# pfnet-research/chainer-differentiable-mpc

Measured on AMD Instinct MI355X. Metric: LQR timestep-solves/sec @ batch=4096 T=50 n_x=8 n_u=2, higher is better.
Workload: dtype f32

## Files before the change

### chainer_differentiable_mpc_amd/csrc/gen_lqr_asm.py

```python
#!/usr/bin/env python
import os

HERE = os.path.dirname(os.path.abspath(__file__))
OUT = os.path.join(HERE, "lqr_asm_gen.hpp")

SHAPES = [(8, 2), (3, 1), (4, 2), (6, 2), (2, 2), (1, 1), (2, 1), (3, 2), (4, 4)]
DB = 3
DF = int(os.environ.get("GEN_FWD_DEPTH", "6"))
KROW = 12
VBASE = 128

X_NO_VMWAIT = os.environ.get("GEN_NO_VMWAIT") == "1"
X_NO_DMA = os.environ.get("GEN_NO_DMA") == "1"
X_NO_LDSREAD = os.environ.get("GEN_NO_LDSREAD") == "1"
X_SKIP_FWD = os.environ.get("GEN_SKIP_FWD") == "1"
X_SKIP_BWD = os.environ.get("GEN_SKIP_BWD") == "1"
X_FWD = set(os.environ.get("GEN_FWD_SKIP", "").split(","))
X_TIMING = os.environ.get("GEN_TIMING") == "1"
X_NEWTON = os.environ.get("GEN_NEWTON") == "1"
X_WARM_STUBS = os.environ.get("GEN_WARM_STUBS") == "1"
X_RET_DIRECT = os.environ.get("GEN_RET_SETPC") != "1"
MFMA_USE = int(os.environ.get("GEN_MFMA_USE", "5"))
MFMA_DEP = int(os.environ.get("GEN_MFMA_DEP", "2"))
X_QP_VALU = os.environ.get("GEN_QP_VALU", "1") == "1"
X_G10_MIX = os.environ.get("GEN_G10_MIX") == "1"
RING_DEPTH = int(os.environ.get("GEN_RING_DEPTH", "3"))
X_NT = set(os.environ.get("GEN_NT", "plain,save,affine,adj").split(","))
USE_MFMA = os.environ.get("GEN_NO_MFMA") != "1"


class Layout:
    def __init__(self, nx, nu, depth=DB, ghbm=False):
        self.nx, self.nu, self.ns = nx, nu, nx + nu
        self.depth = depth
        ns = self.ns
        self.nC, self.nc, self.nF, self.nf = ns * ns, ns, nx * ns, nx
        self.OFF_C = 0
        self.OFF_c = 16 * self.nC
        self.OFF_F = self.OFF_c + 16 * self.nc
        self.OFF_f = self.OFF_F + 16 * self.nF
        self.nchunk_b = self.nC + self.nc + self.nF + self.nf
        self.ndma_b = (self.nchunk_b + 63) // 64
        self.compact = depth > DB
        self.SLOT_B = self.ndma_b * 1024 if not self.compact else (16 * self.nchunk_b + 63) // 64 * 64
        self.last_lanes = (self.SLOT_B - (self.ndma_b - 1) * 1024) // 16
        self.FOFF_f = 16 * self.nF
        self.nG = nu * KROW // 4 * 1 if ghbm else 0
        assert (nu * KROW) % 4 == 0
        self.nG = nu * KROW if ghbm else 0
        self.FOFF_G = 16 * (self.nF + self.nf)
        self.nchunk_f = self.nF + self.nf + self.nG
        self.ndma_f = (self.nchunk_f + 63) // 64
        self.SLOT_F = self.ndma_f * 1024
        deep = RING_DEPTH * ((16 * self.nchunk_b + 63) // 64 * 64) if RING_DEPTH > DB else 0
        self.RING = max(deep, DB * self.ndma_b * 1024, DF * self.SLOT_F)
        assert depth * self.SLOT_B <= self.RING
        assert self.ndma_b * 1024 - 1024 <= 4095 and ns + 1 <= 12 and nu in (1, 2, 3, 4)
        assert (depth - 1) * self.ndma_b <= 63 and (DF - 1) * self.ndma_f <= 63 and 1 <= self.last_lanes <= 64
        self.stash_ok = (64 % nx == 0) and nx <= 8
        self.H = (ns + 1) // 2
        self.stash_pieces = []
        o = 0
        while self.H - o >= 2:
            self.stash_pieces.append((2, o))
            o += 2
        if self.H - o == 1:
            self.stash_pieces.append((1, o))
        self.stash_regs = self.H
        self.NSTASH = min(256 // self.stash_regs - (1 if 256 % self.stash_regs == 0 else 0), 64)
        self.SPD = 64 // nx
        self.NFD = (self.NSTASH + 1 + self.SPD - 1) // self.SPD
        self.FAREA = self.NFD * 1024


# ... 72 lines not shown
                self.trans[w] = 0
            else:
                self.trans.pop(w, None)

    def fmac_dpp(self, acc, a, b, lane):
        self.valu("v_fmac_f32_dpp %s, %s, %s row_newbcast:%d row_mask:0xf bank_mask:0xf" % (acc, a, b, lane),
                  writes=(acc,), reads=(b, acc), dpp=a)

    def mul_dpp(self, dst, a, b, lane):
        self.valu("v_mul_f32_dpp %s, %s, %s row_newbcast:%d row_mask:0xf bank_mask:0xf" % (dst, a, b, lane),
                  writes=(dst,), reads=(b,), dpp=a)

    def mov_dpp(self, dst, a, lane):
        self.valu("v_mov_b32_dpp %s, %s row_newbcast:%d row_mask:0xf bank_mask:0xf" % (dst, a, lane),
                  writes=(dst,), dpp=a)

    def v(self, text, writes=(), reads=(), trans=False):
        self.valu(text, writes=writes, reads=reads, trans=trans)

    def text(self):
        return self.lines


class Regs:
    def __init__(self, base):
        self.next = base

    def take(self, n=1, align=1):
        while self.next % align:
            self.next += 1
        r = list(range(self.next, self.next + n))
        self.next += n
        return ["v%d" % i for i in r]


def vrange(regs):
    a, b = int(regs[0][1:]), int(regs[-1][1:])
    assert b - a + 1 == len(regs)
    return "v[%d:%d]" % (a, b)


def gen_kernel(nx, nu, write_k, stash, masked=False, mpc=False, expand=False, ghbm=False, save=False, affine=False, adj=False):
    D = DB if (masked or mpc) else RING_DEPTH
    kind = "mpc" if mpc else "masked" if masked else "save" if save else "adj" if adj else "affine" if affine else "plain"
    L = Layout(nx, nu, D, ghbm)
    ns, aff = L.ns, L.ns
    assert not stash or L.stash_ok
    assert not ghbm or not (stash or write_k or masked or mpc or save or affine)
    assert not mpc or (masked and write_k and not stash)
    assert not expand or (mpc and 12 * nu + 4 * nx <= 64)
    assert not save or (write_k and not masked and not mpc)
    assert not affine or (stash and not write_k and not masked and not mpc and not save and ns >= 4)
    assert not adj or affine
    P = Prog()
    R = Regs(VBASE)
    ptr = ["%%[ptr%d]" % q for q in range(L.ndma_b)]
    str1 = ["%%[str1_%d]" % q for q in range(L.ndma_b)]
    strd = ["%%[str%d]" % q for q in range(L.ndma_b)]
    aq = ["%%[aq%d]" % i for i in range(ns)]
    af = ["%%[af%d]" % k for k in range(nx)]
    fptr = ["%%[fptr%d]" % q for q in range(2 if adj else L.ndma_f)]
    fstr = ["%%[fstr%d]" % q for q in range(2 if adj else L.ndma_f)]
    fp = ["%%[fp%d]" % q for q in range(L.NFD)]
    pk = ["%%[pk%d]" % m for m in range(nu)]

    mfma = USE_MFMA and ns <= 12 and nx % 4 == 0 and not affine
    NQ = 4 * ((ns + 3) // 4)
    AQX, AQU, AKR = (2, 4, 8) if nu == 2 else (1, 2, 3)
    Q = [R.take(max(ns, AKR + nu) if affine else (NQ if mfma else ns), align=4) for _ in range(3)]
    F = [R.take(nx) for _ in range(3)]
    W = R.take(max(nx, 8 if mpc else 4), align=4)
    G10 = R.take(1)[0]
    A = [R.take(nu, align=4 if save and nu == 2 and m_ == 0 else 1) for m_ in range(nu)]
    SV_Q, SV_U = 16 * nx * (nx + 1), 16 * (nx * (nx + 1) + nx * nu)
    SV_N = nx * (nx + 1) + nx * nu + nu * nu
    SV_NST = (SV_N + 63) // 64
    Kt = R.take(nu)
    Rr = R.take(nu)
    tP, tPQ, tL0, tM1, tRA, tRB, tRP, tT, tLL, tD2, tRD, tY1, tT2 = TMP13 = R.take(13, align=2 if expand else 1)
    MINPIV = R.take(1)[0]
    QB = R.take(1)[0] if affine else None
    XV0 = R.take(1)[0]
    SVD = [R.take(4, align=4) for _ in range(SV_NST)] if save else None
    ACT = [R.take(nu) for _ in range(3)] if masked and not mpc else None
    EPS = R.take(1)[0] if masked and not mpc else None
    UC = [R.take(nu) for _ in range(3)] if mpc else None
    LB = [R.take(nu) for _ in range(3)] if mpc else None
    UB = [R.take(nu) for _ in range(3)] if mpc else None
    XK = R.take(nu) if mpc else None
    QU = R.take(nu) if mpc else None
    NQP = R.take(1)[0] if mpc else None
    QINFO = R.take(1)[0] if mpc else None
    TAU = R.take(3) if expand else None
    Am = [R.take(nu) for _ in range(nu)] if masked else None
    Rm = R.take(nu) if masked else None
    RF = Regs(VBASE)
    M = [RF.take(ns, align=4), RF.take(ns, align=4), RF.take(ns, align=4)]
    ACC = RF.take(4)
    assert RF.next <= int(MINPIV[1:])
    last_vgpr = R.next - 1
    assert last_vgpr <= 255

    def stash_regs_of(p, j):
        base = 0
        for pp in range(p):
            base += L.stash_pieces[pp][0] * L.NSTASH
# ... 355 lines not shown
            P.v("v_cndmask_b32_e32 %s, %s, %s, vcc" % (tRA, rhs[0], rhs[1]), writes=(tRA,), reads=(rhs[0], rhs[1]))
            P.v("v_cndmask_b32_e32 %s, %s, %s, vcc" % (tRB, rhs[1], rhs[0]), writes=(tRB,), reads=(rhs[0], rhs[1]))
            if X_NEWTON:
                P.v("v_fma_f32 %s, -%s, %s, 1.0" % (tT, tP, tRP), writes=(tT,), reads=(tP, tRP))
                P.v("v_fmac_f32_e32 %s, %s, %s" % (tRP, tT, tRP), writes=(tRP,), reads=(tT, tRP))
            P.v("v_mul_f32_e32 %s, %s, %s" % (tLL, tL0, tRP), writes=(tLL,), reads=(tL0, tRP))
            P.v("v_fma_f32 %s, -%s, %s, %s" % (tD2, tLL, tPQ, tM1), writes=(tD2,), reads=(tLL, tPQ, tM1))
            P.v("v_rcp_f32_e32 %s, %s" % (tRD, tD2), writes=(tRD,), reads=(tD2,), trans=True)
            P.v("v_fma_f32 %s, -%s, %s, %s" % (tY1, tLL, tRA, tRB), writes=(tY1,), reads=(tLL, tRA, tRB))
            P.v("v_min3_f32 %s, |%s|, |%s|, %s" % (MINPIV, tP, tD2, MINPIV), writes=(MINPIV,), reads=(tP, tD2, MINPIV))
            if X_NEWTON:
                P.v("v_fma_f32 %s, -%s, %s, 1.0" % (tT, tD2, tRD), writes=(tT,), reads=(tD2, tRD))
                P.v("v_fmac_f32_e32 %s, %s, %s" % (tRD, tT, tRD), writes=(tRD,), reads=(tT, tRD))
            P.raw("s_mov_b64 exec, " + S_KM)
            P.v("v_mul_f32_e64 %s, %s, -%s" % (Kt[1], tY1, tRD), writes=(Kt[1],), reads=(tY1, tRD))
            P.v("v_fma_f32 %s, %s, %s, %s" % (tT2, tPQ, Kt[1], tRA), writes=(tT2,), reads=(tPQ, Kt[1], tRA))
            P.v("v_mul_f32_e64 %s, %s, -%s" % (Kt[0], tT2, tRP), writes=(Kt[0],), reads=(tT2, tRP))
        if mpc:
            for m in range(nu):
                P.v("v_cndmask_b32_e64 %s, %s, %s, %s" % (Kt[m], Kt[m], XK[m], S_AFF), writes=(Kt[m],), reads=(Kt[m], XK[m]))
        if ghbm:
            P.uses(Kt)
            P.raw("s_mov_b64 exec, " + S_GM)
            for m in range(nu):
                P.raw("global_store_dword %%[pgw], %s, off offset:%d" % (Kt[m], m * KROW * 4))
        elif not mpc:
            for m in range(nu):
                off = (" offset:%d" % (m * KROW * 4)) if m else ""
                P.raw("ds_write_b32 %%[ak], %s%s" % (Kt[m], off))
        if write_k:
            P.uses(Kt)
            for m in range(nu):
                P.raw("global_store_dword %s, %s, off" % (pk[m], Kt[m]))
        if save:
            P.uses(Qs[:nx] + [r_ for row_ in A for r_ in row_])
            P.raw("s_mov_b64 exec, " + S_UM)
            for i in range(nx):
                P.raw("ds_write_b32 %%[asq], %s offset:%d" % (Qs[i], SV_Q + i * nu * 4))
            P.raw("s_mov_b64 exec, " + S_ROW0)
            quu = [r_ for row_ in A for r_ in row_]
            if nu == 2 and int(quu[0][1:]) % 4 == 0:
                P.raw("ds_write_b128 %%[asu], %s offset:%d" % (vrange(quu), SV_U))
            else:
                for j_, r_ in enumerate(quu):
                    P.raw("ds_write_b32 %%[asu], %s offset:%d" % (r_, SV_U + 4 * j_))
        P.raw("s_mov_b64 exec, -1")
        P.exec_written()
        if write_k:
            for m in range(nu):
                P.v("v_lshl_add_u64 %s, %s, 0, %%[dk]" % (pk[m], pk[m]))
        if ghbm:
            P.v("v_lshl_add_u64 %[pgw], %[pgw], 0, %[dgw]")
        elif not mpc:
            P.v("v_add_u32_e32 %%[ak], %d, %%[ak]" % ((-nu * KROW * 4) & 0xffffffff))

    def gains_affine(s, first):
        Qs = Q[s]
        QUa, KK = W[0:nu], W[2:2 + nu]
        Aa = [[Qs[AQU + m * nu + l] for l in range(nu)] for m in range(nu)]
        S_PIV = "s[86:87]"
        fact, qch = [], []
        if nu == 1:
            fact.append(lambda: P.v("v_rcp_f32_e32 %s, %s" % (tRP, Aa[0][0]), writes=(tRP,), reads=(Aa[0][0],), trans=True))
            fact.append(lambda: P.v("v_fma_f32 %s, -%s, %s, 1.0" % (tT, Aa[0][0], tRP), writes=(tT,), reads=(Aa[0][0], tRP)))
            fact.append(lambda: P.v("v_fmac_f32_e32 %s, %s, %s" % (tRP, tT, tRP), writes=(tRP,), reads=(tT, tRP)))
        else:
            a00, a01, a10, a11 = Aa[0][0], Aa[0][1], Aa[1][0], Aa[1][1]
            fact.append(lambda: P.v("v_cmp_gt_f32_e64 %s, |%s|, |%s|" % (S_PIV, a10, a00), reads=(a10, a00)))
            fact.append(lambda: P.v("v_cndmask_b32_e64 %s, %s, %s, %s" % (tP, a00, a10, S_PIV), writes=(tP,), reads=(a00, a10)))
            fact.append(lambda: P.v("v_cndmask_b32_e64 %s, %s, %s, %s" % (tL0, a10, a00, S_PIV), writes=(tL0,), reads=(a00, a10)))
            fact.append(lambda: P.v("v_rcp_f32_e32 %s, %s" % (tRP, tP), writes=(tRP,), reads=(tP,), trans=True))
            fact.append(lambda: P.v("v_cndmask_b32_e64 %s, %s, %s, %s" % (tPQ, a01, a11, S_PIV), writes=(tPQ,), reads=(a01, a11)))
            fact.append(lambda: P.v("v_cndmask_b32_e64 %s, %s, %s, %s" % (tM1, a11, a01, S_PIV), writes=(tM1,), reads=(a01, a11)))
            fact.append(lambda: P.v("v_fma_f32 %s, -%s, %s, 1.0" % (tT, tP, tRP), writes=(tT,), reads=(tP, tRP)))
            fact.append(lambda: P.v("v_fmac_f32_e32 %s, %s, %s" % (tRP, tT, tRP), writes=(tRP,), reads=(tT, tRP)))
            fact.append(lambda: P.v("v_mul_f32_e32 %s, %s, %s" % (tLL, tL0, tRP), writes=(tLL,), reads=(tL0, tRP)))
            fact.append(lambda: P.v("v_fma_f32 %s, -%s, %s, %s" % (tD2, tLL, tPQ, tM1), writes=(tD2,), reads=(tLL, tPQ, tM1)))
            fact.append(lambda: P.v("v_rcp_f32_e32 %s, %s" % (tRD, tD2), writes=(tRD,), reads=(tD2,), trans=True))
            fact.append(lambda: P.v("v_fma_f32 %s, -%s, %s, 1.0" % (tT2, tD2, tRD), writes=(tT2,), reads=(tD2, tRD)))
            fact.append(lambda: P.v("v_fmac_f32_e32 %s, %s, %s" % (tRD, tT2, tRD), writes=(tRD,), reads=(tT2, tRD)))
        if not first:
            for k in range(nx):
                if k == 1:
                    qch.append(lambda k=k: P.mul_dpp(QB, G10, F[s][k], k))
                elif k % 2 == 1:
                    qch.append(lambda k=k: P.fmac_dpp(QB, G10, F[s][k], k))
                else:
                    qch.append(lambda k=k: P.fmac_dpp(Qs[0], G10, F[s][k], k))
        while fact or qch:
            if qch:
                qch.pop(0)()
            if fact:
                fact.pop(0)()
        if not first and nx > 1:
            P.v("v_add_f32_e32 %s, %s, %s" % (Qs[0], QB, Qs[0]), writes=(Qs[0],), reads=(QB, Qs[0]))
        for m in range(nu):
            P.mov_dpp(QUa[m], Qs[0], nx + m)
        if nu == 1:
            P.v("v_mul_f32_e64 %s, %s, -%s" % (KK[0], QUa[0], tRP), writes=(KK[0],), reads=(QUa[0], tRP))
        else:
            P.v("v_cndmask_b32_e64 %s, %s, %s, %s" % (tRA, QUa[0], QUa[1], S_PIV), writes=(tRA,), reads=(QUa[0], QUa[1]))
            P.v("v_cndmask_b32_e64 %s, %s, %s, %s" % (tRB, QUa[1], QUa[0], S_PIV), writes=(tRB,), reads=(QUa[0], QUa[1]))
            P.v("v_fma_f32 %s, -%s, %s, %s" % (tY1, tLL, tRA, tRB), writes=(tY1,), reads=(tLL, tRA, tRB))
            P.v("v_mul_f32_e64 %s, %s, -%s" % (KK[1], tY1, tRD), writes=(KK[1],), reads=(tY1, tRD))
            P.v("v_fma_f32 %s, %s, %s, %s" % (tT2, tPQ, KK[1], tRA), writes=(tT2,), reads=(tPQ, KK[1], tRA))
            P.v("v_mul_f32_e64 %s, %s, -%s" % (KK[0], tT2, tRP), writes=(KK[0],), reads=(tT2, tRP))
        P.v("v_fma_f32 %s, %s, %s, %s" % (G10, Qs[AQX], KK[0], Qs[0]), writes=(G10,), reads=(Qs[AQX], KK[0], Qs[0]))
# ... 261 lines not shown
            P.comment("---- backward step, register set %d, ring slot %d" % (k % 3, k % D))
            bstep(k, False)
            P.raw("s_sub_u32 %s, %s, 1" % (S_N, S_N))
            if k != LC:
                P.raw("s_cbranch_scc1 Lbwd_done_%=")
            else:
                P.raw("s_cbranch_scc0 Lbwd_%=")
    P.label("Lbwd_done_%=")
    in_loop[0] = False
    n_bwd = P.n_instr
    if mpc:
        P.v("v_mov_b32_e32 %[xvout], 0")
        P.v("v_mov_b32_e32 %%[nqp], %s" % NQP)
        P.v("v_mov_b32_e32 %%[qpinfo], %s" % QINFO)
        P.raw("s_branch Ldone_%=")

    def read_rows(c, a, aff_too=True):
        if X_NO_LDSREAD and in_loop[0]:
            return
        Mc = M[c]
        if ns % 2 == 0:
            i = 0
            while i + 4 <= ns:
                P.raw("ds_read2_b64 %s, %%[arow] offset0:%d offset1:%d" % (vrange(Mc[i:i + 4]), i // 2, i // 2 + 1))
                i += 4
            if i < ns:
                P.raw("ds_read_b64 %s, %%[arow] offset:%d" % (vrange(Mc[i:i + 2]), i * 4))
        else:
            i = 0
            while i + 2 <= ns:
                P.raw("ds_read2_b32 %s, %%[arow] offset0:%d offset1:%d" % (vrange(Mc[i:i + 2]), i, i + 1))
                i += 2
            if i < ns:
                P.raw("ds_read_b32 %s, %%[arow] offset:%d" % (Mc[i], i * 4))
        if aff_too:
            P.raw("ds_read_b32 %s, %%[aaff]" % ACC[a])

    def fcompute(c, a, ap, mask, last, fillers=()):
        fillers = list(fillers)
        skip = X_FWD if in_loop[0] else set()
        for jj in range(nx):
            if "xpart" not in skip:
                P.fmac_dpp(ACC[a], ACC[ap], M[c][jj], jj)
        if not last:
            for m in range(nu):
                if fillers:
                    fillers.pop(0)()
                if "upart" not in skip:
                    P.fmac_dpp(ACC[a], ACC[a], M[c][nx + m], nx + m)
        for f in fillers:
            f()
        if adj:
            return
        if "store" not in skip:
            P.raw("s_mov_b64 exec, " + mask)
            P.raw("global_store_dword %%[pst], %s, off" % ACC[a])
            P.raw("s_mov_b64 exec, -1")
            P.exec_written()
        if not last and "pst" not in skip:
            P.v("v_lshl_add_u64 %[pst], %[pst], 0, %[dst]")

    P.comment("---- forward rollout")
    stamp(2)
    P.raw("s_waitcnt vmcnt(0) lgkmcnt(0)")
    P.v("v_mov_b32_e32 %[xvout], 0")
    P.raw("v_readfirstlane_b32 %s, %%[bwd_only]" % S_TMP)
    P.raw("s_cmp_lg_u32 %s, 0" % S_TMP)
    P.raw("s_cbranch_scc1 Ldone_%=")
    if not adj:
        P.raw("s_mov_b64 exec, " + S_XM)
        P.raw("global_store_dword %%[px0], %s, off" % XV0)
        P.raw("s_mov_b64 exec, -1")
        P.exec_written()
    if not stash:
        rare = []

        def advance_f():
            if not ghbm:
                advance(fptr, fstr)
                return
            uniq[0] += 1
            lab_r, lab_b = "Lfrare%d_%%=" % uniq[0], "Lfback%d_%%=" % uniq[0]
            P.raw("s_cmp_gt_i32 %s, 1" % S_TF)
            P.raw("s_cbranch_scc0 " + lab_r)
            for p_, s_ in zip(fptr, fstr):
                P.v("v_lshl_add_u64 %s, %s, 0, %s" % (p_, p_, s_))
            P.raw("s_sub_i32 %s, %s, 1" % (S_TF, S_TF))
            P.label(lab_b, reset=False)
            rare.append((lab_r, lab_b))

        P.raw("s_sub_i32 %s, %%[T], %d" % (S_TF, 1 if ghbm else 2))
        for j in range(DF):
            issue_group(fptr, j, L.SLOT_F)
            advance_f()
        P.raw("s_waitcnt vmcnt(%d)" % ((DF - 1) * L.ndma_f))
        read_rows(0, 0)
        P.v("v_mov_b32_e32 %s, %s" % (ACC[2], XV0), writes=(ACC[2],))
        P.raw("s_sub_i32 %s, %%[T], 1" % S_N)
        P.raw("s_cmp_lg_u32 %s, 0" % S_N)
        P.raw("s_cbranch_scc0 Lfin0_%=")
        if X_SKIP_FWD:
            P.raw("s_branch Lfin0_%=")
        in_loop[0] = True
        P.label("Lfwd_%=")
        n_fwd0 = P.n_instr
        for j in range(DF):
            c, a = j % 2, j % 3
            o, an, ap = 1 - c, (a + 1) % 3, (a + 2) % 3
            P.comment("---- forward step, slot %d" % j)
            P.raw("s_waitcnt lgkmcnt(0)")
            issue_group(fptr, j, L.SLOT_F)
            advance_f()
            vmwait((DF - 1) * L.ndma_f)
            d = "2" if j == DF - 1 else ""
            P.v("v_add_u32_e32 %%[arow], %%[drow%s], %%[arow]" % d)
            P.v("v_add_u32_e32 %%[aaff], %%[daff%s], %%[aaff]" % d)
            read_rows(o, an)
            fcompute(c, a, ap, S_SM, False)
            P.raw("s_sub_i32 %s, %s, 1" % (S_N, S_N))
            P.raw("s_cmp_lg_u32 %s, 0" % S_N)
            if j < DF - 1:
                P.raw("s_cbranch_scc0 Lfin%d_%%=" % (j + 1))
            else:
                P.raw("s_cbranch_scc1 Lfwd_%=")
                P.raw("s_branch Lfin0_%=")
        n_fwd = P.n_instr - n_fwd0
        n_fwd_steps = DF
        in_loop[0] = False
        for j in range(DF):
            c, a = j % 2, j % 3
            ap = (a + 2) % 3
            P.label("Lfin%d_%%=" % j)
            P.raw("s_waitcnt lgkmcnt(0)")
            fcompute(c, a, ap, S_UM, True)
            P.v("v_mov_b32_e32 %%[xvout], %s" % ACC[a])
            P.raw("s_branch Ldone_%=")
        for lab_r, lab_b in rare:
            P.label(lab_r, reset=False)
            P.raw("s_cmp_eq_i32 %s, 1" % S_TF)
            P.raw("s_cbranch_scc0 " + lab_b)
            for q_, p_ in enumerate(fptr):
                P.v("v_lshl_add_u64 %s, %s, 0, %%[fstrl%d]" % (p_, p_, q_))
            P.raw("s_sub_i32 %s, %s, 1" % (S_TF, S_TF))
            P.raw("s_branch " + lab_b)
    else:
        def sets(n):
            return n % 3, n % 4, (n + 1) % 4

        def prefetch_a(m, move=True):
            Mc = M[sets(m)[0]]
            if m >= 1 and not ("stage" in X_FWD and in_loop[0]):
                regs = [r for p in range(len(L.stash_pieces)) for r in stash_regs_of(p, m - 1)]
                for jj in range(L.H):
                    P.v("v_accvgpr_read_b32 %s, a%d" % (Mc[jj], regs[jj]), writes=(Mc[jj],))
                for jj in range(L.H):
                    if L.H + jj < ns:
                        P.valu("v_mov_b32_dpp %s, %s row_ror:8 row_mask:0xf bank_mask:0xf" % (Mc[L.H + jj], Mc[jj]),
                               writes=(Mc[L.H + jj],), dpp=Mc[jj])
            if move:
                P.v("v_add_u32_e32 %[arow], %[drowo], %[arow]")
                P.v("v_add_u32_e32 %[aaff], %[daff], %[aaff]")

        def prefetch_b(m):
            c, a, _ = sets(m)
            if "read" in X_FWD and in_loop[0]:
                return
            P.raw("s_mov_b64 exec, " + S_HI)
            read_rows(c, a, aff_too=False)
            P.raw("s_mov_b64 exec, -1")
            P.exec_written()
            P.raw("ds_read_b32 %s, %%[aaff]" % ACC[a])

        def prefetch(m, move=True):
            before = len(P.lines)
            prefetch_a(m, move)
            prefetch_b(m)
            return sum(1 for ln in P.lines[before:] if ln.startswith("ds_"))

        def group_size(m):
            if m < 0:
                return 0
            save = (list(P.lines), P.n_instr, dict(P.age), dict(P.trans))
            k = prefetch(m)
            P.lines, P.n_instr, P.age, P.trans = save
            return k

        if adj:
            DFA = 4
            nVv, nX, nU = nx * (nx + 1), nx, nu
            nda = (nVv + nX + nU + 63) // 64
            SLOTA = nda * 1024
            STG = DFA * SLOTA
            nout = L.nchunk_b
            nst = (nout + 63) // 64
            assert STG + 16 * nout <= L.RING and (DFA - 1) * nda + 4 * nst <= 63
            O_dc, O_dF, O_df = 16 * ns * ns, 16 * (ns * ns + ns), 16 * (ns * ns + ns + nx * ns)
            fixed = set(r_ for grp in M for r_ in grp) | set(ACC) | {MINPIV, XV0} | set(TS)
            pool = ["v%d" % i for i in range(VBASE, 256) if "v%d" % i not in fixed]

            def take(k, align=1):
                for st in range(len(pool)):
                    blk = pool[st:st + k]
                    if len(blk) == k and int(blk[0][1:]) % align == 0 and int(blk[-1][1:]) - int(blk[0][1:]) == k - 1:
                        del pool[st:st + k]
                        return blk
                raise AssertionError("out of forward registers")

            VR = [take(nx, align=2) for _ in range(2)]
            LN = take(2)
            DLN = take(3)
            TAUR = take(3)
            DTAU, HDT, WT, DFV = take(4)
            RC = take(ns)
            RFm = take(nx)
            SD = [take(4, align=4) for _ in range(nst)]
            S_DFSEL = "s[86:87]"

            def load_data(m):
                off = (m % DFA) * SLOTA
                Vs = VR[m % 2]
                av = "%%[avr%d]" % (m % DFA)
                for j in range(0, nx - 1, 2):
                    P.raw("ds_read2_b32 %s, %s offset0:%d offset1:%d" % (vrange(Vs[j:j + 2]), av, j, j + 1))
                if nx % 2:
                    P.raw("ds_read_b32 %s, %s offset:%d" % (Vs[nx - 1], av, (nx - 1) * 4))
                P.raw("ds_read_b32 %s, %s offset:%d" % (LN[m % 2], av, nx * 4))
                P.raw("ds_read_b32 %s, %%[atx] offset:%d" % (TAUR[m % 3], off))

            def issue_data(m):
# ... 101 lines not shown
            stubs = []
            for n in range(1, L.NSTASH + 1):
                P = Prog()
                emit_stub(n)
                stubs.append(P)
            P = P_keep
            FSTUB = 64
            while FSTUB < 8 * max(q.n_instr for q in stubs):
                FSTUB *= 2
            lo = int(S_JMP[2:S_JMP.index(":")])
            P.v("v_cmp_ne_u32_e64 %s, 0, %%[dfshift]" % S_DFSEL)
            P.raw("s_getpc_b64 " + S_JMP)
            P.label("Lpcf_%=", reset=False)
            P.raw("s_sub_i32 %s, %%[T], 2" % S_TMP)
            P.raw("s_mul_i32 %s, %s, %d" % (S_TMP, S_TMP, FSTUB))
            P.raw("s_add_u32 s%d, s%d, Lfstub_%%=-Lpcf_%%=" % (lo, lo))
            P.raw("s_addc_u32 s%d, s%d, 0" % (lo + 1, lo + 1))
            P.raw("s_add_u32 s%d, s%d, %s" % (lo, lo, S_TMP))
            P.raw("s_addc_u32 s%d, s%d, 0" % (lo + 1, lo + 1))
            P.raw("s_setpc_b64 " + S_JMP)
            n_fwd0 = P.n_instr
            for n in range(L.NSTASH, 0, -1):
                c, a, ap = sets(n)
                P.label("Lfs%d_%%=" % n)
                P.raw("s_waitcnt lgkmcnt(0)")
                Vn, ln = VR[(n - 1) % 2], LN[(n - 1) % 2]
                lam = [lambda j=j: P.fmac_dpp(ln, TAUR[(n - 1) % 3], Vn[j], j) for j in range(nx)]
                if n >= 2:
                    data_wait(n)
                    fill = [lambda m=n - 2: prefetch_a(m), lambda m=n - 2: (adj_prefetch_b(m), load_data(m))]
                else:
                    fill = []
                fcompute(c, a, ap, S_SM, False, fill + lam)
                outputs(n, False)
            n_fwd = P.n_instr - n_fwd0
            n_fwd_steps = L.NSTASH
            c, a, ap = sets(0)
            P.raw("s_waitcnt lgkmcnt(0)")
            fcompute(c, a, ap, S_UM, True)
            outputs(0, True)
            P.v("v_mov_b32_e32 %%[xvout], %s" % ACC[a])
            P.raw("s_branch Ldone_%=")
            P.lines.append(".p2align %d" % (FSTUB.bit_length() - 1))
            P.label("Lfstub_%=")
            for q in stubs:
                P.lines.append(".p2align %d" % (FSTUB.bit_length() - 1))
                P.lines += q.lines
                P.n_instr += q.n_instr
        else:
            FSTUB = 64
            while FSTUB < 8 * (2 * (2 * L.H + ns // 2 + 6) + 4):
                FSTUB *= 2
            lo = int(S_JMP[2:S_JMP.index(":")])
            P.raw("s_getpc_b64 " + S_JMP)
            P.label("Lpcf_%=", reset=False)
            P.raw("s_sub_i32 %s, %%[T], 2" % S_TMP)
            P.raw("s_mul_i32 %s, %s, %d" % (S_TMP, S_TMP, FSTUB))
            P.raw("s_add_u32 s%d, s%d, Lfstub_%%=-Lpcf_%%=" % (lo, lo))
            P.raw("s_addc_u32 s%d, s%d, 0" % (lo + 1, lo + 1))
            P.raw("s_add_u32 s%d, s%d, %s" % (lo, lo, S_TMP))
            P.raw("s_addc_u32 s%d, s%d, 0" % (lo + 1, lo + 1))
            P.raw("s_setpc_b64 " + S_JMP)
            n_fwd0 = P.n_instr
            in_loop[0] = True
            for n in range(L.NSTASH, 0, -1):
                c, a, ap = sets(n)
                P.label("Lfs%d_%%=" % n)
                P.raw("s_waitcnt lgkmcnt(%d)" % group_size(n - 1))
                fill = []
                if n >= 2:
                    fill = [lambda m=n - 2: prefetch_a(m), lambda m=n - 2: prefetch_b(m)]
                    if nu == 1:
                        fill = [lambda m=n - 2: prefetch(m)]
                fcompute(c, a, ap, S_SM, False, fill)
            n_fwd = P.n_instr - n_fwd0
            n_fwd_steps = L.NSTASH
            in_loop[0] = False
            c, a, ap = sets(0)
            P.raw("s_waitcnt lgkmcnt(0)")
            fcompute(c, a, ap, S_UM, True)
            P.v("v_mov_b32_e32 %%[xvout], %s" % ACC[a])
            P.raw("s_branch Ldone_%=")
            P.lines.append(".p2align %d" % (FSTUB.bit_length() - 1))
            P.label("Lfstub_%=")
            for n in range(1, L.NSTASH + 1):
                c, a, ap = sets(n)
                P.lines.append(".p2align %d" % (FSTUB.bit_length() - 1))
                prefetch(n, move=False)
                prefetch(n - 1)
                P.v("v_mov_b32_e32 %s, %s" % (ACC[ap], XV0), writes=(ACC[ap],))
                P.raw("s_branch Lfs%d_%%=" % n)
        P.lines.append(".p2align 5")
        P.label("Lbstub_%=")
        for n in range(1, L.NSTASH + 1):
            P.lines.append(".p2align 5")
            for p, (w, off) in enumerate(L.stash_pieces):
                regs = stash_regs_of(p, n - 1)
                if w == 2:
                    P.raw("ds_read2_b32 a[%d:%d], %%[sr%d] offset0:%d offset1:%d" % (regs[0], regs[1], n % D, off, off + 1))
                else:
                    P.raw("ds_read_b32 a%d, %%[sr%d] offset:%d" % (regs[0], n % D, off * 4))
            if X_RET_DIRECT:
                P.raw("s_branch Lret%d_%%=" % (bret["first"] if n == 1 else bret[(n - 2) % LC + 1]))
            else:
                P.raw("s_setpc_b64 " + S_RET)
    P.label("Ldone_%=")
    P.v("v_mov_b32_e32 %%[minpiv], %s" % MINPIV)
    P.raw("s_waitcnt vmcnt(0) lgkmcnt(0)")
    stamp(3)
    for i in range(len(TS)):
        P.v("v_mov_b32_e32 %%[ts%d], %s" % (i, TS[i]))

    outs = [("xvout", '"=&v"(xvout)'), ("minpiv", '"=&v"(minpiv)')]
    if mpc:
        outs += [("nqp", '"=&v"(nqp)'), ("qpinfo", '"=&v"(qpinfo)')]
    if TS:
        outs += [("ts%d" % i, '"=&v"(in.ts[%d])' % i) for i in range(4)]
    rw = []
    for q in range(L.ndma_b):
        rw.append(("ptr%d" % q, '"+v"(in.ptr[%d])' % q))
    NDA = (nx * (nx + 1) + ns + 63) // 64
    NST = (L.nchunk_b + 63) // 64
    assert NDA <= 2
    if not stash or adj:
        for q in range(NDA if adj else L.ndma_f):
            rw.append(("fptr%d" % q, '"+v"(in.fptr[%d])' % q))
    if adj:
        rw.append(("avp", '"+v"(in.avp)'))
        for q in range(NST):
            rw.append(("pso%d" % q, '"+v"(in.pso[%d])' % q))
    rw += [("tf", '"+s"(in.tf)'), ("gz", '"+v"(in.gz)'), ("ak", '"+v"(in.ak)'), ("arow", '"+v"(in.arow)'), ("aaff", '"+v"(in.aaff)'), ("pst", '"+v"(in.pst)')]
    if write_k:
        for m in range(nu):
            rw.append(("pk%d" % m, '"+v"(in.pk[%d])' % m))
    if ghbm:
        rw.append(("pgw", '"+v"(in.pgw)'))
    if masked:
        rw.append(("pm", '"+v"(in.pm)'))
    if save:
        for q in range(SV_NST):
            rw.append(("pso%d" % q, '"+v"(in.pso[%d])' % q))
    ins = []
    for q in range(L.ndma_b):
        ins.append(("str1_%d" % q, '"v"(in.str1[%d])' % q))
        ins.append(("str%d" % q, '"v"(in.str[%d])' % q))
    for i in range(4 if affine else ns):
        ins.append(("aq%d" % i, '"v"(in.aq[%d])' % i))
    for k in range(nx):
        ins.append(("af%d" % k, '"v"(in.af[%d])' % k))
    ins += [("eaff", '"v"(in.eaff)'), ("dst", '"v"(in.dst)'), ("pxi", '"v"(in.pxi)'), ("px0", '"v"(in.px0)')]
    if stash:
        for q in range(L.NFD):
            ins.append(("fp%d" % q, '"v"(in.fp[%d])' % q))
        for q in range(D):
            ins.append(("sr%d" % q, '"v"(in.sr[%d])' % q))
        ins += [("drowo", '"v"(in.drow)'), ("daff", '"v"(in.daff)'),
                ("farea", '"s"(in.farea)')]
    else:
        for q in range(L.ndma_f):
            ins.append(("fstr%d" % q, '"v"(in.fstr[%d])' % q))
        ins += [("drow", '"v"(in.drow)'), ("drow2", '"v"(in.drow2)'), ("daff", '"v"(in.daff)'), ("daff2", '"v"(in.daff2)')]
    if adj:
        for q in range(NDA):
            ins.append(("fstr%d" % q, '"v"(in.fstr[%d])' % q))
        for q in range(NST):
            ins.append(("sso%d" % q, '"v"(in.sso[%d])' % q))
        for q in range(4):
            ins.append(("avr%d" % q, '"v"(in.avr[%d])' % q))
        ins += [("atx", '"v"(in.atx)'), ("awc", '"v"(in.awc)'), ("awe", '"v"(in.awe)'), ("awf", '"v"(in.awf)'),
                ("awd", '"v"(in.awd)'), ("ach", '"v"(in.ach)'), ("wa", '"v"(in.wa)'), ("wb", '"v"(in.wb)'),
                ("dfshift", '"v"(in.dfshift)')]
    if write_k:
        ins.append(("dk", '"v"(in.dk)'))
    if ghbm:
        ins.append(("dgw", '"v"(in.dgw)'))
        for q in range(L.ndma_f):
            ins.append(("fstrl%d" % q, '"v"(in.fstrl[%d])' % q))
    if save:
        for q in range(SV_NST):
            ins.append(("sso%d" % q, '"v"(in.sso[%d])' % q))
        ins += [("asv", '"v"(in.asv)'), ("asq", '"v"(in.asq)'), ("asu", '"v"(in.asu)'), ("ach", '"v"(in.ach)')]
    if masked:
        ins += [("dm", '"v"(in.dm)'), ("am", '"v"(in.am)')]
    ins += [("ring", '"s"(in.ring)'), ("T", '"s"(in.T)'), ("nz", '"s"(in.nz)'), ("bwd_only", '"v"(in.bwd_only)')]
    if mpc:
        ins.append(("nqp_iter", '"s"(in.n_qp_iter)'))
    if expand:
        ins += [("atau", '"v"(in.atau)'), ("act", '"v"(in.act)')]
    clob = ['"v%d"' % i for i in range(VBASE, (255 if adj else last_vgpr) + 1)] + ['"a%d"' % i for i in range(n_agpr)] + \
        ['"s%d"' % i for i in ([70] + list(range(72, 102 if (mpc or affine) else (100 if (save or ghbm) else 98))))] + ['"vcc"', '"scc"', '"memory"']

    tf = lambda b: "true" if b else "false"
    name = "LqrAsm<%d, %d, %s, %s, %s, %s, %s, %s, %s>" % (nx, nu, tf(write_k), tf(stash), tf(masked), tf(ghbm), tf(save), tf(affine), tf(adj))
    if mpc:
        name = "MpcAsm<%d, %d, %s>" % (nx, nu, tf(expand))
    o = []
    o.append("// (%d,%d) write_k=%d stash=%d masked=%d: %d instructions in prologue + 4 backward steps, %d in %d unrolled forward steps\n"
             % (nx, nu, write_k, stash, masked, n_bwd, n_fwd, n_fwd_steps))
    o.append("template <>\nstruct %s {\n" % name)
    o.append("  static constexpr bool kAvailable = true;\n")
    o.append("  static constexpr int NDB = %d, NDF = %d, SLOT_B = %d, SLOT_F = %d, RING_BYTES = %d, KROW = %d, DEPTH_F = %d, DEPTH_B = %d;\n"
             % (L.ndma_b, L.ndma_f, L.SLOT_B, L.SLOT_F, L.RING, KROW, DF, D))
    o.append("  static constexpr int OFF_C = %d, OFF_c = %d, OFF_F = %d, OFF_f = %d, FOFF_f = %d, FOFF_G = %d;\n"
             % (L.OFF_C, L.OFF_c, L.OFF_F, L.OFF_f, L.FOFF_f, L.FOFF_G))
    o.append("  static constexpr int NSTASH = %d, NFD = %d, FAREA_BYTES = %d, HROW = %d, SPD = %d, PADM = %d;\n"
             % (L.NSTASH, L.NFD, L.FAREA, L.H, L.SPD, 16 * L.nchunk_b))
    if adj:
        o.append("  static constexpr int ADJ_NDA = %d, ADJ_SLOT = %d, ADJ_NST = %d;\n" % (NDA, NDA * 1024, NST))
    if save:
        o.append("  static constexpr int SAVE_STAGE_BYTES = %d, SAVE_NST = %d;\n" % (16 * SV_N, SV_NST))
    rw1 = [("ptr%d" % q, '"+v"(in.ptr[%d])' % q) for q in range(L.ndma_b)] + [("tf", '"+s"(in.tf)')]
    if masked:
        rw1.append(("pm", '"+v"(in.pm)'))
    ins1 = []
    for q in range(L.ndma_b):
        ins1.append(("str1_%d" % q, '"v"(in.str1[%d])' % q))
        ins1.append(("str%d" % q, '"v"(in.str[%d])' % q))
    if masked:
        ins1.append(("dm", '"v"(in.dm)'))
    ins1 += [("ring", '"s"(in.ring)'), ("T", '"s"(in.T)')]
    o.append("  static __device__ __forceinline__ void issue_first(LqrAsmIn<%d, %d> &in) {\n" % (nx, nu))
    o.append("    asm volatile(\n")
    for ln in P_first.text():
        o.append('        "%s\\n\\t"\n' % ln)
    o.append("        : " + ", ".join("[%s] %s" % x for x in rw1) + "\n")
    o.append("        : " + ", ".join("[%s] %s" % x for x in ins1) + "\n")
    o.append('        : "scc", "memory");\n')
    o.append("  }\n")
    o.append("  static __device__ __forceinline__ void run(LqrAsmIn<%d, %d> &in, float &xvout, float &minpiv%s) {\n"
             % (nx, nu, ", int &nqp, int &qpinfo" if mpc else ""))
    o.append("    asm volatile(\n")
    for ln in P.text():
        o.append('        "%s\\n\\t"\n' % ln)
    o.append("        : " + ", ".join("[%s] %s" % x for x in outs + rw) + "\n")
    o.append("        : " + ", ".join("[%s] %s" % x for x in ins) + "\n")
    o.append("        : " + ", ".join(clob) + ");\n")
    o.append("  }\n};\n\n")
    return "".join(o)


HEADER = """// lqr_asm_gen.hpp - GENERATED by gen_lqr_asm.py; do not edit.
// Whole-kernel gfx950 instruction streams of the fused LQR solve (lqr/lqr_recursion.py:69-209 of the reference),
// 16-lane row layout, one per (nx, nu, write_k, stash).  The C++ side that prepares the per-lane operands is
// lqr_asm_kernel.hpp.
#pragma once
#include <cstdint>

namespace dmpc {

// per-lane operands of the instruction stream (see lqr_asm_kernel.hpp for how they are filled)
template <int NX, int NU>
struct LqrAsmIn {
  static constexpr int NS = NX + NU;
  // backward sweep
  uint64_t ptr[4], str1[4], str[4];  // LDS-DMA source of this lane's chunk (t = T-1), first / later time strides
  unsigned aq[NS], af[NX];           // LDS byte addresses (ring slot 0) of this lane's [C|c] rows and [F|f] rows
  unsigned ak;                       // LDS byte address of gain row (T-1, 0), this lane's column
  unsigned gz;                       // LDS byte address of this wave's gain rows + lane64 * 16 (zero fill)
  int nz;                            // wave-uniform: 1 KB pieces of the gain rows of one wave
# ... 95 lines not shown
```

### chainer_differentiable_mpc_amd/csrc/lqr_asm_kernel.hpp

```cpp
#pragma once
#include "api_util.hpp"
#include "colwise.hpp"
#include "lqr_asm_gen.hpp"
#include "lqr_dma_kernel.hpp"
#include "lqr_kernels.hpp"

namespace dmpc {

__device__ const float4 dmpc_zero_chunks[16] = {};

template <int NX, int NU, bool STASH, bool SAVE = false, bool GHBM = false>
constexpr size_t lqr_asm_gain_bytes(int T) {
  using G = LqrAsm<NX, NU, false, STASH>;
  if constexpr (GHBM) return 0;
  const size_t rows = (size_t)4 * T * NU * G::KROW * 4, filled = round_up(rows, 1024);
  if constexpr (SAVE) {
    const size_t both = round_up(rows, 16) + (size_t)LqrAsm<NX, NU, true, STASH, false, false, true>::SAVE_STAGE_BYTES;
    return both > filled ? both : filled;
  } else {
    return filled;
  }
}

template <int NX, int NU, bool STASH, bool SAVE = false, bool GHBM = false>
constexpr size_t lqr_asm_lds_bytes(int T) {
  using G = LqrAsm<NX, NU, false, STASH>;
  return (size_t)4 * G::RING_BYTES + (STASH ? (size_t)4 * G::FAREA_BYTES : 0) +
         4 * lqr_asm_gain_bytes<NX, NU, STASH, SAVE, GHBM>(T);
}

template <int NX, int NU, class G, bool HAS_F>
__device__ __forceinline__ void lqr_asm_backward_sources(LqrAsmIn<NX, NU> &in, const float *C, const float *c, const float *F,
                                                         const float *f, int T, size_t B, int b0, int lane64,
                                                         const float *c_u = nullptr) {
  constexpr int NS = NX + NU;
  constexpr int nC = NS * NS, nc = NS, nF = NX * NS, nf = NX;
  const char *Cb = reinterpret_cast<const char *>(C), *cb = reinterpret_cast<const char *>(c);
  const char *Fb = reinterpret_cast<const char *>(F);
  const char *fb = HAS_F ? reinterpret_cast<const char *>(f) : reinterpret_cast<const char *>(dmpc_zero_chunks);
  constexpr size_t per_f = HAS_F ? (size_t)NX * 4 : 0;
  static_assert(nf <= 16, "dmpc_zero_chunks too small");
#pragma unroll
  for (int q = 0; q < 4; ++q) {
    if (q >= G::NDB) {
      in.ptr[q] = in.str1[q] = in.str[q] = 0;
      continue;
    }
    const int g = q * 64 + lane64;
    const bool isC = g < nC, isc = !isC && g < nC + nc, isF = !isC && !isc && g < nC + nc + nF;
    const bool isf = !isC && !isc && !isF && g < nC + nc + nF + nf;
    const bool dyn = isF || isf;
    const bool split = c_u != nullptr, iscu = isc && split && g >= nC + NX;
    const uint64_t base = iscu ? reinterpret_cast<uint64_t>(c_u) : isc ? reinterpret_cast<uint64_t>(cb)
                          : isF ? reinterpret_cast<uint64_t>(Fb) : isf ? reinterpret_cast<uint64_t>(fb)
                          : reinterpret_cast<uint64_t>(Cb);
    const size_t per = iscu ? (size_t)NU * 4 : isc ? (split ? (size_t)NX * 4 : (size_t)NS * 4) : isF ? (size_t)NX * NS * 4
                       : isf ? per_f : (size_t)NS * NS * 4;
    const int g0 = isC ? 0 : iscu ? nC + NX : isc ? nC : isF ? nC + nc : isf ? nC + nc + nF : g;
    const size_t off = (size_t)(g - g0) * 16;
    const int t0 = dyn ? T - 2 : T - 1;
    const uint64_t p = base + ((size_t)t0 * B + (size_t)b0) * per + off;
    in.ptr[q] = p - (uint64_t)q * 1024u;
    const uint64_t s = (uint64_t)0 - (uint64_t)(B * per);
    in.str[q] = s;
    in.str1[q] = dyn ? 0 : s;
  }
}

template <int NX, int NU, class G>
__device__ __forceinline__ void lqr_asm_affine_sources(LqrAsmIn<NX, NU> &in, const float *Ks, const float *Qxu, const float *Quu,
                                                       const float *c, const float *F, int T, size_t B, int b0, int lane64,
                                                       const float *c_u = nullptr) {
  constexpr int NS = NX + NU;
  constexpr int nC = NS * NS, nc = NS, nF = NX * NS, nf = NX;
  constexpr int nK = NU * NX, nQx = NX * NU, nQu = NU * NU;
  static_assert(nK + nQx + nQu <= nC, "the saved blocks fit the C region");
  const uint64_t zero = reinterpret_cast<uint64_t>(dmpc_zero_chunks);
#pragma unroll
  for (int q = 0; q < 4; ++q) {
// ... 76 lines not shown
  const int T = a.T;
  const size_t B = (size_t)a.B;
  const int wave = __builtin_amdgcn_readfirstlane((int)threadIdx.x >> 6);
  const int lane64 = threadIdx.x & 63;
  const int r = lane64 >> 4;
  const int lane = lane64 & 15;
  int b0 = ((int)blockIdx.x * 4 + wave) * 4;
  if (b0 > a.B - 4) b0 = a.B - 4;
  b0 = __builtin_amdgcn_readfirstlane(b0);
  const int b = b0 + r;

  extern __shared__ float lds[];
  const unsigned lds0 = lds_byte_address(lds);
  const unsigned ring = lds0 + (unsigned)wave * G::RING_BYTES;
  const unsigned farea = lds0 + 4u * G::RING_BYTES + (unsigned)wave * (STASH ? G::FAREA_BYTES : 0);
  const unsigned gain_wave_bytes = (unsigned)lqr_asm_gain_bytes<NX, NU, STASH, SAVE, GHBM>(T);
  const unsigned gain_wave = lds0 + 4u * G::RING_BYTES + (STASH ? 4u * G::FAREA_BYTES : 0u) + (unsigned)wave * gain_wave_bytes;
  const unsigned gain_traj = gain_wave + (unsigned)r * (unsigned)(T * NU * KROW * 4);

  LqrAsmIn<NX, NU> in;
  in.ring = __builtin_amdgcn_readfirstlane(ring);
  in.T = T;
  in.tf = 0;
  in.bwd_only = (a.x == nullptr && !ADJ) ? 1 : 0;

  if constexpr (AFFINE) lqr_asm_affine_sources<NX, NU, G>(in, a.Ks_in, a.Qxu_in, a.Quu_in, a.c, a.F, T, B, b0, lane64, a.c_u);
  else lqr_asm_backward_sources<NX, NU, G, HAS_F>(in, a.C, a.c, a.F, a.f, T, B, b0, lane64, a.c_u);
  const char *Fb = reinterpret_cast<const char *>(a.F);
  const char *fb = HAS_F ? reinterpret_cast<const char *>(a.f) : reinterpret_cast<const char *>(dmpc_zero_chunks);
  constexpr size_t per_f = HAS_F ? (size_t)NX * 4 : 0;
  if constexpr (MASKED) {
    in.pm = reinterpret_cast<uint64_t>(a.mask) + ((size_t)(T - 1) * B + (size_t)b0) * NU + (size_t)(lane64 < NU ? lane64 : 0) * 4 -
            (uint64_t)G::PADM;
    in.dm = (uint64_t)0 - (uint64_t)(B * NU);
    in.am = ring + (unsigned)(r * NU);
  } else {
    in.pm = in.dm = 0;
    in.am = 0;
  }
  G::issue_first(in);
  in.gz = gain_wave + (unsigned)lane64 * 16u;
  in.nz = GHBM ? 0 : (int)(round_up((size_t)4 * T * NU * KROW * 4, 1024) / 1024u);
  if constexpr (GHBM) {
    const size_t tb = (size_t)(T - 1) * B + (size_t)b;
    in.pgw = reinterpret_cast<uint64_t>(a.wsK + tb * NU * KROW + (lane <= NS ? lane : NS));
    in.dgw = (uint64_t)0 - (uint64_t)(B * NU * KROW * 4);
  } else {
    in.pgw = in.dgw = 0;
  }
  const int lane_c = lane < NS ? lane : NS - 1;
  const bool col_aff = lane == AFF;
  if constexpr (AFFINE) lqr_asm_affine_addresses<NX, NU, G>(in, ring, r, lane, a.c_u != nullptr);
  else lqr_asm_row_addresses<NX, NU, G>(in, ring, r, lane, a.c_u != nullptr);
  in.ak = gain_traj + (unsigned)((T - 1) * NU * KROW * 4) + (unsigned)lane * 4u;
  in.eaff = col_aff ? 1.f : 0.f;
  if constexpr (WRITE_K) {
    const size_t tb = (size_t)(T - 1) * B + (size_t)b;
#pragma unroll
    for (int m = 0; m < NU; ++m)
      in.pk[m] = col_aff ? reinterpret_cast<uint64_t>(a.ks + tb * NU + m)
                         : reinterpret_cast<uint64_t>(a.Ks + (tb * NU + m) * NX + (lane < NX ? lane : 0));
    in.dk = (uint64_t)0 - (uint64_t)(col_aff ? B * NU * 4 : B * NU * NX * 4);
  } else {
#pragma unroll
    for (int m = 0; m < NU; ++m) in.pk[m] = 0;
    in.dk = 0;
  }
  if constexpr (SAVE) {
    constexpr int nVv = NX * (NX + 1), nQx = NX * NU, nQu = NU * NU;
    const unsigned stg = gain_wave + (unsigned)round_up((size_t)4 * T * NU * KROW * 4, 16);
    const int m_ = lane >= NX && lane < NS ? lane - NX : 0;
    in.asv = stg + (unsigned)((r * NX * (NX + 1) + (lane < NX ? lane : NX)) * 4);
    in.asq = stg + (unsigned)((r * NX * NU + m_) * 4);
    in.asu = stg + (unsigned)(r * NU * NU * 4);
    in.ach = stg + (unsigned)lane64 * 16u;
#pragma unroll
    for (int q = 0; q < 4; ++q) {
      const int g = q * 64 + lane64;
      const bool isV = g < nVv, isQx = !isV && g < nVv + nQx, isQu = !isV && !isQx && g < nVv + nQx + nQu;
      const uint64_t base = isV ? reinterpret_cast<uint64_t>(a.Vv_out) : isQx ? reinterpret_cast<uint64_t>(a.Qxu_out)
                                                                              : reinterpret_cast<uint64_t>(a.Quu_out);
      const size_t per = isV ? (size_t)NX * (NX + 1) * 4 : isQx ? (size_t)NX * NU * 4 : (size_t)NU * NU * 4;
      const int g0 = isV ? 0 : isQx ? nVv : nVv + nQx;
      const bool any = isV || isQx || isQu;
      in.pso[q] = any ? base + ((size_t)(T - 1) * B + (size_t)b0) * per + (size_t)(g - g0) * 16 : 0;
      in.sso[q] = any ? (uint64_t)0 - (uint64_t)(B * per) : 0;
    }
  } else {
    in.asv = in.asq = in.asu = 0;
  }

  const bool row_x = lane < NX;
  const int m_own = row_x ? 0 : (lane < NS ? lane - NX : NU - 1);
  const unsigned arow_u = gain_traj + (unsigned)(m_own * KROW * 4);
#pragma unroll
  for (int q = 0; q < 2; ++q) in.fptr[q] = in.fstr[q] = in.fstrl[q] = 0;
#pragma unroll
  for (int q = 0; q < 8; ++q) in.fp[q] = 0;
  {
    const int i8 = (lane & 7) < NX ? (lane & 7) : NX - 1;
    const unsigned half_row = (unsigned)(G::OFF_F + ((r * NX + i8) * NS + (lane >> 3) * G::HROW) * 4);
#pragma unroll
    for (int q = 0; q < 6; ++q) in.sr[q] = q < G::DEPTH_B ? ring + (unsigned)(q * G::SLOT_B) + half_row : 0u;
  }
  in.farea = __builtin_amdgcn_readfirstlane(farea);
  if constexpr (STASH) {
    static_assert(G::NFD <= 8 && 64 % NX == 0, "f area layout");
#pragma unroll
    for (int q = 0; q < G::NFD; ++q) {
      int tt = q * G::SPD + lane64 / NX;
      if (tt > T - 2) tt = T - 2;
      in.fp[q] = reinterpret_cast<uint64_t>(fb) + ((size_t)tt * B + (size_t)b0) * per_f + (size_t)(lane64 % NX) * 16;
    }
    in.arow = arow_u;
    in.aaff = row_x ? farea + (unsigned)((r * NX + lane) * 4) : arow_u + (unsigned)(NS * 4);
    in.drow = (unsigned)(NU * KROW * 4);
    in.drow2 = in.drow;
    in.daff = row_x ? (unsigned)(NX * 16) : (unsigned)(NU * KROW * 4);
    in.daff2 = in.daff;
  } else {
#pragma unroll
    for (int q = 0; q < 2; ++q) {
      if (q >= G::NDF) continue;
      const int g = q * 64 + lane64;
      const char *base = Fb;
      size_t per = (size_t)NX * NS * 4, off = 0;
      if (g < nF) {
        off = (size_t)g * 16;
      } else if (g < nF + nf) {
        base = fb; per = per_f; off = (size_t)(g - nF) * 16;
      } else if (GHBM && g < nF + nf + NU * KROW) {
        base = reinterpret_cast<const char *>(a.wsK); per = (size_t)NU * KROW * 4; off = (size_t)(g - nF - nf) * 16;
      }
      in.fptr[q] = reinterpret_cast<uint64_t>(base) + (size_t)b0 * per + off - (uint64_t)q * 1024u;
      in.fstr[q] = (uint64_t)(B * per);
      in.fstrl[q] = (GHBM && g >= nF + nf && g < nF + nf + NU * KROW) ? (uint64_t)(B * per) : 0;
    }
    const unsigned arow_g = GHBM ? ring + (unsigned)(G::FOFF_G + (r * NU + m_own) * KROW * 4) : arow_u;
    in.arow = row_x ? ring + (unsigned)((r * NX + lane) * NS * 4) : arow_g;
    in.aaff = row_x ? ring + (unsigned)(G::FOFF_f + (r * NX + lane) * 4) : arow_g + (unsigned)(NS * 4);
    in.drow = (row_x || GHBM) ? (unsigned)G::SLOT_F : (unsigned)(NU * KROW * 4);
    in.drow2 = (row_x || GHBM) ? (unsigned)G::SLOT_F - (unsigned)(G::DEPTH_F * G::SLOT_F) : (unsigned)(NU * KROW * 4);
    in.daff = in.drow;
    in.daff2 = in.drow2;
  }
  in.pst = row_x ? reinterpret_cast<uint64_t>(a.x + (B + (size_t)b) * NX + lane)
                 : reinterpret_cast<uint64_t>(a.u + (size_t)b * NU + m_own);
  in.dst = row_x ? (uint64_t)(B * NX * 4) : (uint64_t)(B * NU * 4);
  in.pxi = a.x_init != nullptr ? reinterpret_cast<uint64_t>(a.x_init + (size_t)b * NX + (row_x ? lane : NX - 1))
                               : reinterpret_cast<uint64_t>(dmpc_zero_chunks);
  in.px0 = reinterpret_cast<uint64_t>(a.x + (size_t)b * NX + (row_x ? lane : NX - 1));
  if constexpr (ADJ) {
    constexpr int nVv = NX * (NX + 1), nOutC = NS * NS, nOutc = NS, nOutF = NX * NS, nOutf = NX;
    const int lane_x = row_x ? lane : NX - 1;
    in.px0 = reinterpret_cast<uint64_t>(a.dx0 + (size_t)b * NX + lane_x);
    in.avp = farea + (unsigned)((T - 1) * NX * 16 + (r * NX + lane_x) * 4);
#pragma unroll
    for (int q = 0; q < 4; ++q) in.avr[q] = ring + (unsigned)(q * G::ADJ_SLOT + (r * NX + lane_x) * (NX + 1) * 4);
    in.atx = ring + (lane_c < NX ? (unsigned)(nVv * 16 + (r * NX + lane_c) * 4)
                                  : (unsigned)((nVv + NX) * 16 + (r * NU + lane_c - NX) * 4));
    in.awc = ring + (unsigned)((r * NS * NS + lane_c) * 4);
    in.awe = ring + (unsigned)((r * NS + lane_c) * 4);
    in.awf = ring + (unsigned)((r * NX * NS + lane_c) * 4);
    in.awd = ring + (unsigned)((r * NX + lane_x) * 4);
    in.ach = ring + (unsigned)lane64 * 16u;
    in.wa = a.w_a;
    in.wb = a.w_b;
    in.dfshift = a.df_shift;
#pragma unroll
    for (int q = 0; q < 2; ++q) {
      if (q >= G::ADJ_NDA) continue;
// ... 59 lines not shown
```

Measured before the change: 5.722 billion.

## Index stashed gain rows by step in forward rollout using immediate LDS offsets

The backward pass now stores gains ascending in LDS rather than descending. The forward rollout then reads each step's gain row with ds_read at compile-time immediate offsets from a fixed base, so the per-step VGPR pointer increments are gone. For nx divisible by 4, the u-columns of the gain matrix are zeroed once and kept zero via DPP bank masks, which shortens the vector reads. Unmasked x-stores in non-last steps drop the exec save and restore. In exchange the code adds an alignment directive and NOPs, and the layout becomes more complex and limited to offsets that fit in 16 bits.

```diff
diff --git a/chainer_differentiable_mpc_amd/csrc/gen_lqr_asm.py b/chainer_differentiable_mpc_amd/csrc/gen_lqr_asm.py
--- a/chainer_differentiable_mpc_amd/csrc/gen_lqr_asm.py
+++ b/chainer_differentiable_mpc_amd/csrc/gen_lqr_asm.py
@@ -20,6 +20,7 @@
 X_NEWTON = os.environ.get("GEN_NEWTON") == "1"
 X_WARM_STUBS = os.environ.get("GEN_WARM_STUBS") == "1"
 X_RET_DIRECT = os.environ.get("GEN_RET_SETPC") != "1"
+X_ROLL_OLD = os.environ.get("GEN_ROLLOUT") == "old"
 MFMA_USE = int(os.environ.get("GEN_MFMA_USE", "5"))
 MFMA_DEP = int(os.environ.get("GEN_MFMA_DEP", "2"))
 X_QP_VALU = os.environ.get("GEN_QP_VALU", "1") == "1"
@@ -198,6 +199,10 @@
     assert not save or (write_k and not masked and not mpc)
     assert not affine or (stash and not write_k and not masked and not mpc and not save and ns >= 4)
     assert not adj or affine
+    roll_new = stash and kind in ("plain", "save") and not X_ROLL_OLD
+    zero_kept = roll_new and nx % 4 == 0
+    assert not zero_kept or nx in (4, 8)
+    assert not roll_new or (L.NSTASH * nu + nu) * KROW * 4 <= 0xffff
     P = Prog()
     R = Regs(VBASE)
     ptr = ["%%[ptr%d]" % q for q in range(L.ndma_b)]
@@ -659,7 +664,7 @@
         if ghbm:
             P.v("v_lshl_add_u64 %[pgw], %[pgw], 0, %[dgw]")
         elif not mpc:
-            P.v("v_add_u32_e32 %%[ak], %d, %%[ak]" % ((-nu * KROW * 4) & 0xffffffff))
+            P.v("v_add_u32_e32 %%[ak], %d, %%[ak]" % ((nu * KROW * 4 if roll_new else -nu * KROW * 4) & 0xffffffff))
 
     def gains_affine(s, first):
         Qs = Q[s]
@@ -1027,7 +1032,9 @@
             f()
         if adj:
             return
-        if "store" not in skip:
+        if "store" not in skip and roll_new and not last:
+            P.raw("global_store_dword %%[pst], %s, off" % ACC[a])
+        elif "store" not in skip:
             P.raw("s_mov_b64 exec, " + mask)
             P.raw("global_store_dword %%[pst], %s, off" % ACC[a])
             P.raw("s_mov_b64 exec, -1")
@@ -1130,26 +1137,42 @@
                     P.v("v_accvgpr_read_b32 %s, a%d" % (Mc[jj], regs[jj]), writes=(Mc[jj],))
                 for jj in range(L.H):
                     if L.H + jj < ns:
-                        P.valu("v_mov_b32_dpp %s, %s row_ror:8 row_mask:0xf bank_mask:0xf" % (Mc[L.H + jj], Mc[jj]),
+                        bank = (1 << (nx // 4)) - 1 if zero_kept and L.H + jj >= nx else 0xf
+                        P.valu("v_mov_b32_dpp %s, %s row_ror:8 row_mask:0xf bank_mask:0x%x" % (Mc[L.H + jj], Mc[jj], bank),
                                writes=(Mc[L.H + jj],), dpp=Mc[jj])
-            if move:
+            if move and not roll_new:
                 P.v("v_add_u32_e32 %[arow], %[drowo], %[arow]")
                 P.v("v_add_u32_e32 %[aaff], %[daff], %[aaff]")
 
-        def prefetch_b(m):
+        def prefetch_b(m, move=True):
             c, a, _ = sets(m)
             if "read" in X_FWD and in_loop[0]:
                 return
             P.raw("s_mov_b64 exec, " + S_HI)
-            read_rows(c, a, aff_too=False)
+            if roll_new:
+                read_gain_row(c, m)
+            else:
+                read_rows(c, a, aff_too=False)
             P.raw("s_mov_b64 exec, -1")
             P.exec_written()
+            if move and roll_new:
+                P.v("v_add_u32_e32 %[aaff], %[daff], %[aaff]")
             P.raw("ds_read_b32 %s, %%[aaff]" % ACC[a])
+
+        def read_gain_row(c, m):
+            if X_NO_LDSREAD and in_loop[0]:
+                return
+            ncol = nx if zero_kept else ns
+            base, i = m * nu * KROW * 4, 0
+            while i < ncol:
+                w = min(ncol - i, 4)
+                P.raw("ds_read_b%d %s, %%[arow] offset:%d" % (32 * w, vrange(M[c][i:i + w]) if w > 1 else M[c][i], base + i * 4))
+                i += w
 
         def prefetch(m, move=True):
             before = len(P.lines)
             prefetch_a(m, move)
-            prefetch_b(m)
+            prefetch_b(m, move)
             return sum(1 for ln in P.lines[before:] if ln.startswith("ds_"))
 
         def group_size(m):
@@ -1357,6 +1380,10 @@
             while FSTUB < 8 * (2 * (2 * L.H + ns // 2 + 6) + 4):
                 FSTUB *= 2
             lo = int(S_JMP[2:S_JMP.index(":")])
+            if zero_kept:
+                for Mc in M:
+                    for j in range(nx, ns):
+                        P.v("v_mov_b32_e32 %s, 0" % Mc[j], writes=(Mc[j],))
             P.raw("s_getpc_b64 " + S_JMP)
             P.label("Lpcf_%=", reset=False)
             P.raw("s_sub_i32 %s, %%[T], 2" % S_TMP)
@@ -1368,9 +1395,12 @@
             P.raw("s_setpc_b64 " + S_JMP)
             n_fwd0 = P.n_instr
             in_loop[0] = True
+            if roll_new:
+                P.lines.append(".p2align 3")
             for n in range(L.NSTASH, 0, -1):
                 c, a, ap = sets(n)
-                P.label("Lfs%d_%%=" % n)
+                P.comment("---- forward step n = %d" % n)
+                P.label("Lfs%d_%%=" % n, reset=not roll_new)
                 P.raw("s_waitcnt lgkmcnt(%d)" % group_size(n - 1))
                 fill = []
                 if n >= 2:
@@ -1382,6 +1412,7 @@
             n_fwd_steps = L.NSTASH
             in_loop[0] = False
             c, a, ap = sets(0)
+            P.comment("---- forward step n = 0 (u only)")
             P.raw("s_waitcnt lgkmcnt(0)")
             fcompute(c, a, ap, S_UM, True)
             P.v("v_mov_b32_e32 %%[xvout], %s" % ACC[a])
@@ -1394,6 +1425,8 @@
                 prefetch(n, move=False)
                 prefetch(n - 1)
                 P.v("v_mov_b32_e32 %s, %s" % (ACC[ap], XV0), writes=(ACC[ap],))
+                if roll_new:
+                    P.nop(2)
                 P.raw("s_branch Lfs%d_%%=" % n)
         P.lines.append(".p2align 5")
         P.label("Lbstub_%=")
@@ -1459,8 +1492,7 @@
             ins.append(("fp%d" % q, '"v"(in.fp[%d])' % q))
         for q in range(D):
             ins.append(("sr%d" % q, '"v"(in.sr[%d])' % q))
-        ins += [("drowo", '"v"(in.drow)'), ("daff", '"v"(in.daff)'),
-                ("farea", '"s"(in.farea)')]
+        ins += ([] if roll_new else [("drowo", '"v"(in.drow)')]) + [("daff", '"v"(in.daff)'), ("farea", '"s"(in.farea)')]
     else:
         for q in range(L.ndma_f):
             ins.append(("fstr%d" % q, '"v"(in.fstr[%d])' % q))
@@ -1510,6 +1542,7 @@
              % (L.OFF_C, L.OFF_c, L.OFF_F, L.OFF_f, L.FOFF_f, L.FOFF_G))
     o.append("  static constexpr int NSTASH = %d, NFD = %d, FAREA_BYTES = %d, HROW = %d, SPD = %d, PADM = %d;\n"
              % (L.NSTASH, L.NFD, L.FAREA, L.H, L.SPD, 16 * L.nchunk_b))
+    o.append("  static constexpr bool GAIN_BY_N = %s;\n" % tf(roll_new))
     if adj:
         o.append("  static constexpr int ADJ_NDA = %d, ADJ_SLOT = %d, ADJ_NST = %d;\n" % (NDA, NDA * 1024, NST))
     if save:
diff --git a/chainer_differentiable_mpc_amd/csrc/lqr_asm_kernel.hpp b/chainer_differentiable_mpc_amd/csrc/lqr_asm_kernel.hpp
--- a/chainer_differentiable_mpc_amd/csrc/lqr_asm_kernel.hpp
+++ b/chainer_differentiable_mpc_amd/csrc/lqr_asm_kernel.hpp
@@ -24,7 +24,7 @@
 
 template <int NX, int NU, bool STASH, bool SAVE = false, bool GHBM = false>
 constexpr size_t lqr_asm_lds_bytes(int T) {
-  using G = LqrAsm<NX, NU, false, STASH>;
+  using G = LqrAsm<NX, NU, false, STASH, false, GHBM>;
   return (size_t)4 * G::RING_BYTES + (STASH ? (size_t)4 * G::FAREA_BYTES : 0) +
          4 * lqr_asm_gain_bytes<NX, NU, STASH, SAVE, GHBM>(T);
 }
@@ -207,7 +207,7 @@
   const bool col_aff = lane == AFF;
   if constexpr (AFFINE) lqr_asm_affine_addresses<NX, NU, G>(in, ring, r, lane, a.c_u != nullptr);
   else lqr_asm_row_addresses<NX, NU, G>(in, ring, r, lane, a.c_u != nullptr);
-  in.ak = gain_traj + (unsigned)((T - 1) * NU * KROW * 4) + (unsigned)lane * 4u;
+  in.ak = gain_traj + (G::GAIN_BY_N ? 0u : (unsigned)((T - 1) * NU * KROW * 4)) + (unsigned)lane * 4u;
   in.eaff = col_aff ? 1.f : 0.f;
   if constexpr (WRITE_K) {
     const size_t tb = (size_t)(T - 1) * B + (size_t)b;
@@ -268,10 +268,11 @@
       in.fp[q] = reinterpret_cast<uint64_t>(fb) + ((size_t)tt * B + (size_t)b0) * per_f + (size_t)(lane64 % NX) * 16;
     }
     in.arow = arow_u;
-    in.aaff = row_x ? farea + (unsigned)((r * NX + lane) * 4) : arow_u + (unsigned)(NS * 4);
+    const unsigned k0 = G::GAIN_BY_N ? (unsigned)((T - 1) * NU * KROW * 4) : 0u;
+    in.aaff = row_x ? farea + (unsigned)((r * NX + lane) * 4) : arow_u + k0 + (unsigned)(NS * 4);
     in.drow = (unsigned)(NU * KROW * 4);
     in.drow2 = in.drow;
-    in.daff = row_x ? (unsigned)(NX * 16) : (unsigned)(NU * KROW * 4);
+    in.daff = row_x ? (unsigned)(NX * 16) : G::GAIN_BY_N ? 0u - (unsigned)(NU * KROW * 4) : (unsigned)(NU * KROW * 4);
     in.daff2 = in.daff;
   } else {
 #pragma unroll
```

New measurement: 5.719 billion. No clear change (-0.0%).
